# chaoyang223/UDA

Measured on AMD Instinct MI355X. Metric: TeraSort shuffle+merge GB/s whole-node, higher is better.
Workload: dtype bytes

## Files before the change

csrc/gpu/device_engine.cc:

```cpp
#include "device_engine.h"
#include "codec/colpack.h"
#include "device_ptr.h"
#include "hbm_ledger.h"
#include "merge_plan.h"
#include "sdma.h"
#include "uda/fault.h"
#include "uda/topology.h"
#include "uda/trace.h"

#include <rccl/rccl.h>
#include <unistd.h>

#include <algorithm>
#include <atomic>
#include <chrono>
#include <cstring>
#include <map>
#include <mutex>
#include <numeric>
#include <stdexcept>

#include "uda/log.h"
#include "uda/vint.h"
#include "uda/thread_name.h"
// ... 675 lines not shown
  HIP_CHECK(hipStreamWaitEvent(s, pb.planned, 0));
  KwayDesc kd = kp.kd;
  static const bool prof = std::getenv("UDA_KWAY_PROF") != nullptr;
  if (prof) {
    auto ensure = [](DeviceBuffer& b, size_t bytes) {
      if (b.size() < bytes) b.alloc_local(bytes + bytes / 8);
    };
    ensure(kw_prof_, (size_t)kp.ncells * 5 * 8);
    HIP_CHECK(hipMemsetAsync(kw_prof_.as(), 0, (size_t)kp.ncells * 5 * 8, s));
    kd.prof = kw_prof_.as<unsigned long long>();
  }
  HIP_CHECK(hipGetLastError());
  launch_kway_tiles(kd, kp.ncells, out, s);
  HIP_CHECK(hipGetLastError());
  HIP_CHECK(hipEventRecord(pb.used, s));
  pb.used_valid = true;
  if (prof) report_kway_phases(kd.prof, kp.ncells, s);
  last_passes_ = 1;
  return kp.total;
}

ShuffleJob::ShuffleJob(const ShuffleConfig& cfg) : cfg_(cfg) {
  if (cfg_.world < 1 || cfg_.rank < 0 || cfg_.rank >= cfg_.world)
    throw std::runtime_error("ShuffleJob: bad rank/world");
  if (cfg_.maps_per_rank < 1) throw std::runtime_error("ShuffleJob: maps_per_rank < 1");
  if (cfg_.rounds < 1) cfg_.rounds = 1;
  if (cfg_.reducers < 1) cfg_.reducers = 1;
  if (cfg_.pinned_slots < 2) cfg_.pinned_slots = 2;
  if (cfg_.d2h != "sdma" && cfg_.d2h != "hip") throw std::runtime_error("ShuffleJob: d2h must be sdma or hip");
  if (cfg_.store != "hbm" && cfg_.store != "host" && cfg_.store != "disk")
    throw std::runtime_error("unknown store tier " + cfg_.store);
  if (cfg_.delivery_pack != "auto" && cfg_.delivery_pack != "off")
    throw std::runtime_error("ShuffleJob: delivery_pack must be auto or off");
  pack_ = cfg_.deliver_host && cfg_.delivery_pack == "auto";
  if (const char* e = std::getenv("UDA_DELIVERY_PACK"))
    if (std::atoi(e) == 0) pack_ = false;
  R_ = cfg_.reducers;
  Q_ = cfg_.rounds;
  C_ = R_ * Q_;
  if ((int64_t)R_ * cfg_.world * cfg_.maps_per_rank > 65536)
    throw std::runtime_error("ShuffleJob: reducers * world * maps_per_rank must be <= 65536 (merge run index)");
  HIP_CHECK(hipSetDevice(cfg_.device));
  int lo_prio = 0, hi_prio = 0;
  HIP_CHECK(hipDeviceGetStreamPriorityRange(&lo_prio, &hi_prio));
  const bool spill = cfg_.store != "hbm";
  HIP_CHECK(hipStreamCreateWithPriority(&s_comm_, hipStreamNonBlocking, spill ? lo_prio : hi_prio));
  HIP_CHECK(hipStreamCreateWithPriority(&s_compute_, hipStreamNonBlocking, spill ? hi_prio : lo_prio));
  HIP_CHECK(hipStreamCreateWithFlags(&s_copy_, hipStreamNonBlocking));
  HIP_CHECK(hipStreamCreateWithFlags(&s_plan_, hipStreamNonBlocking));
  buf_records_ = std::max<int64_t>(1, cfg_.kv_buf_bytes / kTeraRecordBytes);
  const int64_t buf_bytes = buf_records_ * kTeraRecordBytes;
  piece_bytes_ = std::max<int64_t>(1, cfg_.d2h_piece_bytes / buf_bytes) * buf_bytes;
  ring_stride_ = pack_ ? std::max(piece_bytes_, colpack_bound(kTeraRecordBytes, piece_bytes_ / kTeraRecordBytes))
                       : piece_bytes_;
  merged_ev_.resize(kSlots);
  comm_ev_.resize(kSlots);
  sent_ev_.resize(2);
  for (auto& e : merged_ev_) HIP_CHECK(hipEventCreateWithFlags(&e, hipEventDisableTiming));
  for (auto& e : comm_ev_) HIP_CHECK(hipEventCreateWithFlags(&e, hipEventDisableTiming));
  for (auto& e : sent_ev_) HIP_CHECK(hipEventCreateWithFlags(&e, hipEventDisableTiming));
}

ShuffleJob::~ShuffleJob() {
  {
    std::lock_guard<std::mutex> g(mu_);
    stop_ = true;
// ... 15 lines not shown
    ring_ = nullptr;
    sdma_.reset();
  }
  exchange_.reset();
  if (s_copy_) (void)hipStreamDestroy(s_copy_);
  if (s_plan_) (void)hipStreamDestroy(s_plan_);
  if (s_comm_) (void)hipStreamDestroy(s_comm_);
  if (s_compute_) (void)hipStreamDestroy(s_compute_);
}

void ShuffleJob::init_comm(const std::string& uid) {
  if (cfg_.world == 1) return;
  HIP_CHECK(hipSetDevice(cfg_.device));
  exchange_ = make_rccl_exchange(cfg_.rank, cfg_.world, uid);
}

void ShuffleJob::init_local() {
  if (cfg_.world == 1) return;
  if (cfg_.local_group.empty()) throw std::runtime_error("init_local: config.local_group is empty");
  HIP_CHECK(hipSetDevice(cfg_.device));
  exchange_ = make_local_exchange(cfg_.local_group, cfg_.rank, cfg_.world);
}

void ShuffleJob::init_ipc(const std::string& name) {
  if (cfg_.world == 1) return;
  HIP_CHECK(hipSetDevice(cfg_.device));
  exchange_ = make_ipc_exchange(name, cfg_.rank, cfg_.world, cfg_.device);
}

std::string ShuffleJob::delivery_name() const {
  if (!cfg_.deliver_host) return "none";
  std::string name = sdma_ ? sdma_->describe() : "hip[numa=" + std::to_string(device_numa_node(cfg_.device)) + "]";
  name += " ring=" + ring_numa_;
  if (!pack_) return name + " pack=off";
  name += " pack=colbits";
  if (last_d2h_ratio_ >= 0) {
    char b[32];
    std::snprintf(b, sizeof(b), " d2h/in=%.3f", last_d2h_ratio_);
    name += b;
  }
  return name;
}

std::vector<ShuffleJob::PackPiece> ShuffleJob::round_pieces(const std::vector<int64_t>& group_recs) const {
  std::vector<PackPiece> v;
  int64_t goff = 0, doff = 0;
  for (int i = 0; i < R_; ++i) {
    const int64_t bytes = group_recs[i] * kTeraRecordBytes;
    for (int64_t off = 0; off < bytes;) {
      const int64_t len = std::min(piece_bytes_, bytes - off);
      const int64_t nrec = len / kTeraRecordBytes;
      v.push_back(PackPiece{goff + off, doff, nrec});
      doff += colpack_bound(kTeraRecordBytes, nrec);
      off += len;
    }
    goff += bytes;
  }
  return v;
}

void ShuffleJob::generate() {
  HIP_CHECK(hipSetDevice(cfg_.device));
  const int M = cfg_.maps_per_rank, W = cfg_.world;
  const int nruns = M * W;
  run_off_.assign(nruns, 0);
  run_nrec_.assign(nruns, 0);
// ... 576 lines not shown
      piece_sig_.resize(cfg_.pinned_slots);
      for (auto& sg : piece_sig_) sg = sdma_->make_signal();
    } else {
      ring_ = static_cast<uint8_t*>(hip_host_alloc_on_node(ring_bytes, device_numa_node(cfg_.device)));
      piece_ev_.resize(cfg_.pinned_slots);
      for (auto& e : piece_ev_) HIP_CHECK(hipEventCreateWithFlags(&e, hipEventDisableTiming));
    }
    for (size_t o = 0; o < ring_bytes; o += 4096) ring_[o] = 0;
    ring_numa_ = numa_residency(ring_);
    pinned_free_.assign(cfg_.pinned_slots, true);
    items_.assign(R_, {});
    eof_bufs_.clear();
    for (int i = 0; i < R_; ++i) eof_bufs_.emplace_back(new uint8_t[(size_t)cfg_.kv_buf_bytes + 16]);
    unpack_bufs_.clear();
    if (pack_) {
      const size_t one = (size_t)std::max(cfg_.kv_buf_bytes, buf_records_ * kTeraRecordBytes) + 16;
      for (int i = 0; i < R_; ++i) unpack_bufs_.emplace_back(new uint8_t[2 * one]);
    }
    copy_thr_ = std::thread([this] { name_thread("uda-copy"); copy_loop(); });
    for (int i = 0; i < R_; ++i) consumers_.emplace_back([this, i] { name_thread("uda-consume"); consume_loop(i); });
  }
  UDA_LOG(kInfo, "rank %d planned %d reducers x %d rounds, max round %ld records, delivery %s", cfg_.rank, R_, Q_,
          (long)max_round_records_, delivery_name().c_str());
}

void ShuffleJob::wait_exchange_ok() {
  if (exchange_) exchange_->check();
}

void ShuffleJob::copy_loop() {
  try {
    bind_thread_to_cpus(device_consumer_cpus(cfg_.device));
    HIP_CHECK(hipSetDevice(cfg_.device));
    for (;;) {
      RoundOut r;
      {
        std::unique_lock<std::mutex> lk(mu_);
        cv_.wait(lk, [&] { return stop_ || !round_q_.empty(); });
        if (stop_) return;
        r = std::move(round_q_.front());
        round_q_.pop_front();
      }
      HIP_CHECK(hipEventSynchronize(merged_ev_[r.slot]));
      const uint8_t* src = out_slots_[r.slot].as<uint8_t>();
      const bool last_round = (r.q == Q_ - 1);
      bool check;
      {
        std::lock_guard<std::mutex> g(mu_);
        check = step_check_delivery_;
      }
      if (check) {
        std::vector<RunDesc> gr(R_);
        int64_t o = 0, mx = 0;
        for (int i = 0; i < R_; ++i) {
          gr[i].base = src + o * kTeraRecordBytes;
          gr[i].nrec = r.group_recs[i];
          gr[i].nbytes = gr[i].nrec * kTeraRecordBytes;
          gr[i].offsets = nullptr;
          o += r.group_recs[i];
          mx = std::max(mx, r.group_recs[i]);
        }
        std::vector<uint64_t> ck(R_, 0);
        HIP_CHECK(hipMemcpyAsync(d_d2h_runs_.as(), gr.data(), (size_t)R_ * sizeof(RunDesc), hipMemcpyHostToDevice, s_copy_));
        launch_slice_checksums(d_d2h_runs_.as<RunDesc>(), R_, std::max<int64_t>(mx, 1),
                               d_d2h_ck_.as<unsigned long long>(), s_copy_);
        HIP_CHECK(hipGetLastError());
        HIP_CHECK(hipMemcpyAsync(ck.data(), d_d2h_ck_.as(), (size_t)R_ * 8, hipMemcpyDeviceToHost, s_copy_));
        HIP_CHECK(hipStreamSynchronize(s_copy_));
        std::lock_guard<std::mutex> g(mu_);
        for (int i = 0; i < R_; ++i) pre_d2h_ck_[(size_t)r.q * R_ + i] = ck[i];
      }
      std::vector<int> used;
      int64_t goff = 0;
      const std::vector<PackPiece> ppieces = pack_ ? round_pieces(r.group_recs) : std::vector<PackPiece>();
      const ColpackResult* pres = pack_ ? h_pack_results_[r.slot].as<ColpackResult>() : nullptr;
      size_t pi = 0;
      for (int i = 0; i < R_; ++i) {
        const int64_t bytes = r.group_recs[i] * kTeraRecordBytes;
        if (bytes == 0 && last_round) {
          {
            std::lock_guard<std::mutex> g(mu_);
            items_[i].push_back(Item{-1, 0, true, now_ms(), r.q});
          }
          cv_.notify_all();
        }
        for (int64_t off = 0; off < bytes;) {
          const int64_t len = std::min(piece_bytes_, bytes - off);
          int k = -1;
          {
            std::unique_lock<std::mutex> lk(mu_);
            cv_.wait(lk, [&] {
              if (stop_) return true;
              for (bool f : pinned_free_)
                if (f) return true;
              return false;
            });
            if (stop_) return;
            for (int x = 0; x < (int)pinned_free_.size(); ++x)
              if (pinned_free_[x]) {
                k = x;
                break;
              }
            pinned_free_[k] = false;
          }
          uint8_t* dst = ring_ + (int64_t)k * ring_stride_;
          const uint8_t* from = src + goff + off;
          int64_t copy_len = len;
          bool packed = false;
          if (pack_) {
            if (pi >= ppieces.size() || ppieces[pi].src_off != goff + off || ppieces[pi].nrec * kTeraRecordBytes != len)
              throw std::runtime_error("delivery_pack: piece list out of step with the copy loop");
            const ColpackResult pr = pres[pi];
            if (pr.packed) {
              if (pr.bytes < (int64_t)kColpackHeaderBytes || pr.bytes > colpack_bound(kTeraRecordBytes, ppieces[pi].nrec))
                throw std::runtime_error("delivery_pack: packed length outside the piece's region");
              packed = true;
              copy_len = pr.bytes;
              from = packed_slots_[r.slot].as<uint8_t>() + ppieces[pi].dst_off;
            }
            ++pi;
          }
          if (sdma_) {
            SdmaEngine::arm(piece_sig_[k], sdma_->parts((size_t)copy_len, cfg_.d2h_engines));
            sdma_->copy_d2h(dst, from, (size_t)copy_len, piece_sig_[k], cfg_.d2h_engines);
          } else {
            HIP_CHECK(hipMemcpyAsync(dst, from, (size_t)copy_len, hipMemcpyDeviceToHost, s_copy_));
            HIP_CHECK(hipEventRecord(piece_ev_[k], s_copy_));
          }
          off += len;
          used.push_back(k);
          {
            std::lock_guard<std::mutex> g(mu_);
            items_[i].push_back(Item{k, len, last_round && off >= bytes, now_ms(), r.q, packed, copy_len});
            step_d2h_bytes_ += copy_len;
            ++(packed ? step_packed_ : step_raw_);
          }
          cv_.notify_all();
        }
        goff += bytes;
      }
      for (int k : used) {
        if (sdma_)
          SdmaEngine::wait(piece_sig_[k]);
        else
          HIP_CHECK(hipEventSynchronize(piece_ev_[k]));
      }
      {
        std::lock_guard<std::mutex> g(mu_);
        out_free_[r.q] = 1;
      }
      cv_.notify_all();
    }
  } catch (const std::exception& e) {
    std::lock_guard<std::mutex> g(mu_);
    if (step_error_msg_.empty()) step_error_msg_ = std::string("delivery copy thread: ") + e.what();
    stop_ = true;
    cv_.notify_all();
  }
}

void ShuffleJob::consume_loop(int i) {
  try {
    bind_thread_to_cpus(device_consumer_cpus(cfg_.device));
    HIP_CHECK(hipSetDevice(cfg_.device));
    const int64_t buf_bytes = buf_records_ * kTeraRecordBytes;
    uint8_t* eb = eof_bufs_[i].get();
    const size_t unpack_one = (size_t)std::max(cfg_.kv_buf_bytes, buf_bytes) + 16;
    int64_t unpack_turn = 0;
    for (;;) {
      Item it;
      bool check;
      {
        std::unique_lock<std::mutex> lk(mu_);
        cv_.wait(lk, [&] { return stop_ || !items_[i].empty(); });
        if (stop_) return;
        it = items_[i].front();
        items_[i].pop_front();
        check = step_check_delivery_;
      }
      uint64_t got_ck = 0;
      int err = 0;
      int64_t nb = 0;
      double waited = 0;
      bool eof_sent = false;
      double unpack_ms = 0;
      if (it.pslot >= 0) {
        if (sdma_)
          SdmaEngine::wait(piece_sig_[it.pslot]);
        else
          HIP_CHECK(hipEventSynchronize(piece_ev_[it.pslot]));
        waited = now_ms() - it.issued_ms;
        const uint8_t* base = ring_ + (int64_t)it.pslot * ring_stride_;
        ColpackPiece pp;
        if (it.packed) {
          const char* why = "";
          if (!colpack_open(base, it.copied, kTeraRecordBytes, it.bytes / kTeraRecordBytes, &pp, &why) || !pp.packed)
            throw std::runtime_error(std::string("packed piece rejected: ") + (pp.hdr ? "not marked packed" : why));
        }
        if (check && !it.packed)
          for (int64_t off = 0; off + kTeraRecordBytes <= it.bytes; off += kTeraRecordBytes)
            got_ck += record_hash(base + off, kTeraRecordBytes);
        for (int64_t off = 0; off < it.bytes; off += buf_bytes) {
          const int64_t len = std::min(buf_bytes, it.bytes - off);
          const bool final_chunk = it.last && off + len >= it.bytes;
          if (it.packed) {
            uint8_t* stg = unpack_bufs_[i].get() + (size_t)(unpack_turn++ & 1) * unpack_one;
            if (check || (sink_ && !err)) {
              const double tu = now_ms();
              colpack_unpack(pp, off / kTeraRecordBytes, len / kTeraRecordBytes, stg);
              unpack_ms += now_ms() - tu;
            }
            if (check)
              for (int64_t o = 0; o + kTeraRecordBytes <= len; o += kTeraRecordBytes)
                got_ck += record_hash(stg + o, kTeraRecordBytes);
            if (final_chunk && len + kEofBytes <= cfg_.kv_buf_bytes) {
              stg[len] = 0xFF;
              stg[len + 1] = 0xFF;
              if (sink_ && !err) err = sink_(i, stg, len + kEofBytes);
              eof_sent = true;
            } else if (sink_ && !err) {
              err = sink_(i, stg, len);
            }
            ++nb;
            continue;
          }
          if (final_chunk && len + kEofBytes <= cfg_.kv_buf_bytes) {
            std::memcpy(eb, base + off, (size_t)len);
            eb[len] = 0xFF;
            eb[len + 1] = 0xFF;
            if (sink_ && !err) err = sink_(i, eb, len + kEofBytes);
            eof_sent = true;
          } else if (sink_ && !err) {
            err = sink_(i, base + off, len);
          }
          ++nb;
        }
      }
      if (it.last && !eof_sent) {
        eb[0] = 0xFF;
        eb[1] = 0xFF;
        if (sink_ && !err) err = sink_(i, eb, kEofBytes);
        ++nb;
      }
      {
        std::lock_guard<std::mutex> g(mu_);
        if (it.pslot >= 0) pinned_free_[it.pslot] = true;
        if (check && it.q >= 0 && it.q < Q_) delivered_ck_[(size_t)it.q * R_ + i] += got_ck;
        step_buffers_ += nb;
        step_d2h_ms_ += waited;
        step_unpack_ms_ += unpack_ms;
        if (err && !step_error_) step_error_ = err;
        if (it.last) ++eof_count_;
      }
      cv_.notify_all();
    }
  } catch (const std::exception& e) {
    std::lock_guard<std::mutex> g(mu_);
    if (step_error_msg_.empty()) step_error_msg_ = std::string("delivery consumer thread: ") + e.what();
    stop_ = true;
    cv_.notify_all();
  }
}

void ShuffleJob::refresh_plan() {
  const int M = cfg_.maps_per_rank, W = cfg_.world;
  const int nruns = M * W;
  const int64_t per = C_ + 1;
  for_run_batches([&](int r0, int nr, uint8_t* const* bases, const int64_t* nrec, const int* bset) {
    launch_split_fixed(bases, nrec, C_ > 1 ? d_bounds_.as<Elem>() : nullptr, bset, nr, C_ - 1,
                       d_split_out_.as<int64_t>() + (size_t)r0 * per, s_compute_);
  });
  std::vector<int64_t> pos((size_t)nruns * per);
  HIP_CHECK(hipMemcpyAsync(pos.data(), d_split_out_.as(), pos.size() * 8, hipMemcpyDeviceToHost, s_compute_));
  HIP_CHECK(hipStreamSynchronize(s_compute_));
  if (pos != split_pos_) throw std::runtime_error("replan: the map outputs changed since plan()");
  if (W == 1) return;
  const size_t n_per_peer = (size_t)Q_ * R_ * M;
  std::vector<int64_t> send((size_t)W * n_per_peer), recv((size_t)W * n_per_peer);
  for (int p = 0; p < W; ++p)
    for (int q = 0; q < Q_; ++q)
      for (int i = 0; i < R_; ++i)
        for (int m = 0; m < M; ++m) {
          const int r = m * W + p, c = i * Q_ + q;
          send[(size_t)p * n_per_peer + ((size_t)q * R_ + i) * M + m] = pos[(size_t)r * per + c + 1] - pos[(size_t)r * per + c];
        }
// ... 46 lines not shown
        ++st.pre_d2h_errors;
        note(first[3], "output slot changed between the merge and its D2H", q, i, pre_d2h[(size_t)q * R_ + i], merged);
      }
      if (deliv[(size_t)q * R_ + i] != merged) {
        ++st.delivery_errors;
        note(first[4], "consumer received other bytes than the merge wrote", q, i, deliv[(size_t)q * R_ + i], merged);
      }
    }
  }
  st.diag.clear();
  for (const auto& f : first)
    if (!f.empty()) st.diag += (st.diag.empty() ? "" : "; ") + f;
}

StepStats ShuffleJob::run_step(bool validate) {
  trace::Range tr_step("uda.step");
  HIP_CHECK(hipSetDevice(cfg_.device));
  if (!merger_) throw std::runtime_error("run_step before plan()");
  StepStats st;
  st.validated = validate;
  const double t0 = now_ms();
  const int M = cfg_.maps_per_rank, W = cfg_.world, me = cfg_.rank;
  const bool deliver = cfg_.deliver_host;
  {
    std::lock_guard<std::mutex> g(mu_);
    if (stop_) throw std::runtime_error("delivery pipeline stopped: " + step_error_msg_);
    out_free_.assign(Q_, 0);
    eof_count_ = 0;
    step_buffers_ = 0;
    step_error_ = 0;
    step_d2h_ms_ = 0;
    step_d2h_bytes_ = step_packed_ = step_raw_ = 0;
    step_unpack_ms_ = 0;
    step_check_delivery_ = validate && cfg_.check_delivery && deliver;
    pre_d2h_ck_.assign((size_t)Q_ * R_, 0);
    delivered_ck_.assign((size_t)Q_ * R_, 0);
  }
  std::vector<hipEvent_t> ev(4 * (size_t)Q_);
  for (auto& e : ev) HIP_CHECK(hipEventCreate(&e));
  unsigned long long* vstats = d_validate_.as<unsigned long long>();
  Elem* vprev = reinterpret_cast<Elem*>(d_validate_.as<uint8_t>() + 64);
  Elem* vlast = vprev + R_;
  std::vector<bool> has_prev(R_, false);
  if (validate) {
    HIP_CHECK(hipMemsetAsync(d_validate_.as(), 0, 64, s_compute_));
    HIP_CHECK(hipMemsetAsync(d_diag_.as(), 0, (size_t)Q_ * diag_stride() * 8, s_compute_));
  }
  if (cfg_.replan) {
    const double tp = now_ms();
    refresh_plan();
    st.plan_ms = now_ms() - tp;
  }

  auto wait_until = [&](const std::function<bool()>& ready) {
    std::unique_lock<std::mutex> lk(mu_);
    while (!cv_.wait_for(lk, std::chrono::milliseconds(100), [&] { return ready() || stop_; })) {
      if (exchange_) {
        lk.unlock();
        wait_exchange_ok();
        lk.lock();
      }
    }
    if (stop_) throw std::runtime_error("delivery pipeline failed: " + step_error_msg_);
  };

  const bool staged_send = W > 1 && spilled();
// ... 230 lines not shown
        if (g > 0) {
          launch_validate_fixed(out + goff * kTeraRecordBytes, g, vprev + i, has_prev[i] ? 1 : 0, vlast + i, vstats,
                                s_compute_, dg + 4 + i);
          HIP_CHECK(hipMemcpyAsync(vprev + i, vlast + i, sizeof(Elem), hipMemcpyDeviceToDevice, s_compute_));
          has_prev[i] = true;
        }
        goff += g;
      }
      check_inputs(1);
    }
    HIP_CHECK(hipEventRecord(ev[4 * q + 3], s_compute_));
    if (pack_ && deliver && pack_n_[q] > 0) {
      launch_colpack(d_pack_pieces_[q].as<ColpackPieceDesc>(), pack_n_[q], pack_max_nrec_[q], kTeraRecordBytes,
                     buf_records_, d_pack_table_.as<uint32_t>(), d_pack_results_[slot].as<ColpackResult>(), s_compute_);
      HIP_CHECK(hipGetLastError());
      HIP_CHECK(hipMemcpyAsync(h_pack_results_[slot].as(), d_pack_results_[slot].as(),
                               (size_t)pack_n_[q] * sizeof(ColpackResult), hipMemcpyDeviceToHost, s_compute_));
    }
    HIP_CHECK(hipEventRecord(merged_ev_[slot], s_compute_));
    if (sdma_stage) {
      std::lock_guard<std::mutex> g(mu_);
      merge_recorded[q] = 1;
      cv_.notify_all();
    }
    st.records += n;
    if (deliver) {
      {
        std::lock_guard<std::mutex> g(mu_);
        round_q_.push_back(RoundOut{q, slot, rp.group_recs});
      }
      cv_.notify_all();
    }
  }
  if (deliver) wait_until([&] { return eof_count_ == R_; });
  if (exchange_) exchange_->wait(s_comm_);
  HIP_CHECK(hipStreamSynchronize(s_compute_));
  HIP_CHECK(hipStreamSynchronize(s_comm_));
  HIP_CHECK(hipStreamSynchronize(s_copy_));
  if (stage_thr.joinable()) stage_thr.join();
  if (exchange_) exchange_->quiesce();
  st.wall_ms = now_ms() - t0;
  st.stage_ms = stage_ms;
  for (int q = 0; q < Q_; ++q) {
    float a = 0, b = 0;
    if (staged() && hipEventElapsedTime(&a, ev[4 * q + 0], ev[4 * q + 1]) == hipSuccess) st.comm_ms += a;
    if (hipEventElapsedTime(&b, ev[4 * q + 2], ev[4 * q + 3]) == hipSuccess) st.merge_ms += b;
    st.round_comm_ms.push_back(a);
    st.round_merge_ms.push_back(b);
  }
  static const bool round_trace = std::getenv("UDA_ROUND_TRACE") != nullptr;
  if (round_trace && staged()) {
    std::string line = "[round trace ms: comm start-end | merge start-end]";
    for (int q = 0; q < Q_; ++q) {
      float t[4] = {0, 0, 0, 0};
      for (int k = 0; k < 4; ++k) (void)hipEventElapsedTime(&t[k], ev[0], ev[4 * q + k]);
      char b[96];
      snprintf(b, sizeof(b), " q%d %.0f-%.0f|%.0f-%.0f", q, t[0], t[1], t[2], t[3]);
      line += b;
    }
    fprintf(stderr, "%s\n", line.c_str());
  }
  for (auto e : ev) (void)hipEventDestroy(e);
  st.d2h_ms = step_d2h_ms_;
  st.bytes_in = st.records * kTeraRecordBytes;
  st.buffers = step_buffers_;
  {
    std::lock_guard<std::mutex> g(mu_);
    st.d2h_bytes = step_d2h_bytes_;
    st.packed_pieces = step_packed_;
    st.raw_pieces = step_raw_;
    st.unpack_ms = step_unpack_ms_;
  }
  if (deliver && st.bytes_in > 0) last_d2h_ratio_ = (double)st.d2h_bytes / (double)st.bytes_in;
  if (validate) {
    unsigned long long v[3];
    HIP_CHECK(hipMemcpy(v, vstats, sizeof(v), hipMemcpyDeviceToHost));
    st.order_errors = (int64_t)v[0];
    st.checksum = v[1];
    st.exchange_errors = W > 1 ? (int64_t)v[2] : 0;
    localize_mismatch(st);
  }
  st.bad_layout = merger_->bad_layout();
  if (step_error_) throw std::runtime_error("delivery sink reported error " + std::to_string(step_error_));
  return st;
}

}
}
```

csrc/gpu/device_engine.h:

```cpp
#pragma once
#include <hip/hip_runtime.h>

#include <atomic>
#include <condition_variable>
#include <cstdint>
#include <deque>
#include <functional>
#include <map>
#include <memory>
#include <mutex>
#include <string>
#include <thread>
#include <vector>

#include "exchange.h"
#include "kernels.h"
#include "disk_store.h"
#include "sdma.h"

namespace uda {
namespace gpu {

void hip_check(hipError_t e, const char* what, const char* file, int line);
#define HIP_CHECK(x) ::uda::gpu::hip_check((x), #x, __FILE__, __LINE__)
#define HIP_PENDING(where) ::uda::gpu::hip_check(hipGetLastError(), "a call before " where, __FILE__, __LINE__)

class DeviceBuffer {
 public:
  DeviceBuffer() = default;
  explicit DeviceBuffer(size_t bytes, bool resident = false) { alloc(bytes, resident); }
  ~DeviceBuffer();
  DeviceBuffer(const DeviceBuffer&) = delete;
  DeviceBuffer& operator=(const DeviceBuffer&) = delete;
  DeviceBuffer(DeviceBuffer&& o) noexcept { take(o); }
  DeviceBuffer& operator=(DeviceBuffer&& o) noexcept {
    if (this != &o) {
      reset();
      take(o);
    }
    return *this;
  }
  void alloc(size_t bytes, bool resident = false) { alloc_impl(bytes, resident, true); }
  void alloc_local(size_t bytes) { alloc_impl(bytes, false, false); }
  void reset();
  template <typename T = uint8_t>
  T* as() const {
    return reinterpret_cast<T*>(ptr_);
// ... 138 lines not shown
  PlanBufs pbufs_[2];
  int next_pslot_ = 0;
  std::vector<Slot> slots_;
  int next_slot_ = 0;
  int last_passes_ = 0;
  size_t slot_bytes_ = 0;
};

using SinkFn = std::function<int(int reducer, const uint8_t* buf, int64_t len)>;

struct ShuffleConfig {
  int device = 0;
  int rank = 0;
  int world = 1;
  int maps_per_rank = 32;
  int64_t records_per_map = 1 << 20;
  int rounds = 8;
  int reducers = 1;
  uint64_t seed = 0x5eed;
  int64_t kv_buf_bytes = 1 << 20;
  int64_t d2h_piece_bytes = 128ll << 20;
  int pinned_slots = 16;
  int d2h_engines = 1;
  std::string d2h = "sdma";
  bool deliver_host = true;
  bool validate = false;
  std::string local_group;
  std::string store = "hbm";
  std::string local_dirs;
  bool replan = false;
  bool map_sort = false;
  bool check_delivery = false;
  std::string delivery_pack = "auto";
};

struct StepStats {
  double wall_ms = 0;
  double comm_ms = 0;
  double merge_ms = 0;
  double d2h_ms = 0;
  double wait_out_ms = 0;
  double plan_ms = 0;
  double stage_ms = 0;
  int64_t bytes_in = 0;
  int64_t records = 0;
  int64_t bytes_sent = 0;
  int64_t bytes_h2d = 0;
  int64_t buffers = 0;
  int64_t d2h_bytes = 0;
  int64_t packed_pieces = 0;
  int64_t raw_pieces = 0;
  double unpack_ms = 0;
  int merge_passes = 0;
  bool validated = false;
  int64_t order_errors = -1;
  uint64_t checksum = 0;
  int64_t exchange_errors = -1;
  bool bad_layout = false;
  int64_t pre_merge_errors = -1;
  int64_t own_errors = -1;
  int64_t merge_errors = -1;
  int64_t pre_d2h_errors = -1;
  int64_t delivery_errors = -1;
  std::string diag;
  std::vector<double> round_comm_ms, round_merge_ms;
};

class ShuffleJob {
 public:
  explicit ShuffleJob(const ShuffleConfig& cfg);
  ~ShuffleJob();

  const ShuffleConfig& config() const { return cfg_; }
  void init_comm(const std::string& uid);
  void init_local();
  void init_ipc(const std::string& name);
  void generate();
  std::vector<std::vector<uint64_t>> sample_keys(int64_t every);
  void set_bounds(const std::vector<uint64_t>& bounds);
  void plan();
  void set_sink(SinkFn sink) { sink_ = std::move(sink); }
  StepStats run_step(bool validate);
  void refresh_plan();

  std::vector<uint64_t> local_dest_checksums() const { return dest_checksum_; }
// ... 116 lines not shown
  std::string ring_numa_;
  std::vector<hsa_signal_t> piece_sig_;
  std::vector<hipEvent_t> piece_ev_;
  struct RoundOut {
    int q;
    int slot;
    std::vector<int64_t> group_recs;
  };
  struct Item {
    int pslot;
    int64_t bytes;
    bool last;
    double issued_ms;
    int q;
    bool packed = false;
    int64_t copied = 0;
  };
  std::mutex mu_;
  std::condition_variable cv_;
  std::deque<RoundOut> round_q_;
  std::vector<std::deque<Item>> items_;
  std::vector<bool> pinned_free_;
  std::vector<int> out_free_;
  std::thread copy_thr_;
  std::vector<std::thread> consumers_;
  bool stop_ = false;
  int eof_count_ = 0;
  int64_t step_buffers_ = 0;
  int step_error_ = 0;
  std::string step_error_msg_;
  double step_d2h_ms_ = 0;
  int64_t step_d2h_bytes_ = 0, step_packed_ = 0, step_raw_ = 0;
  double step_unpack_ms_ = 0;
  SinkFn sink_;
  std::vector<std::unique_ptr<uint8_t[]>> eof_bufs_;
  std::vector<std::unique_ptr<uint8_t[]>> unpack_bufs_;
};

std::string nccl_unique_id();
int device_count();

hipStream_t pooled_stream(int priority = 0);
int64_t device_guard_violations();
void return_stream(hipStream_t s);
void prewarm_streams(int device, int n);

}
}
```

csrc/gpu/sdma.cc:

```cpp
#include "sdma.h"
#include "uda/topology.h"

#include <hip/hip_runtime.h>
#include <sched.h>
#include <sys/mman.h>
#include <sys/syscall.h>
#include <unistd.h>

#include <algorithm>
#include <cstdio>
#include <cstdlib>
#include <cstring>
#include <fstream>
#include <sstream>
#include <stdexcept>
#include <mutex>
#include <thread>
#include <atomic>
#include <map>
#include <unordered_map>
#include <vector>

#include "uda/log.h"

// ... 455 lines not shown
    hsa_check(s, "agents_allow_access");
  }
  return p;
}

void SdmaEngine::free_host(void* p) {
  if (!p) return;
  PinnedShare ps;
  if (pinned_share_of(p, 1, &ps))
    pinned_host_free(p);
  else
    (void)hsa_amd_memory_pool_free(p);
}

hsa_signal_t SdmaEngine::make_signal() {
  hsa_signal_t s;
  hsa_check(hsa_signal_create(0, 0, nullptr, &s), "signal_create");
  return s;
}

void SdmaEngine::destroy_signal(hsa_signal_t s) {
  if (s.handle) (void)hsa_signal_destroy(s);
}

void SdmaEngine::arm(hsa_signal_t s, int64_t parts) { hsa_signal_store_screlease(s, parts); }
void SdmaEngine::add(hsa_signal_t s, int64_t parts) { hsa_signal_add_screlease(s, parts); }

void SdmaEngine::wait(hsa_signal_t s) {
  const hsa_signal_value_t v =
      hsa_signal_wait_scacquire(s, HSA_SIGNAL_CONDITION_LT, 1, UINT64_MAX, HSA_WAIT_STATE_BLOCKED);
  if (v < 0) throw std::runtime_error("SDMA copy reported an error (completion signal < 0)");
}

int SdmaEngine::parts(size_t bytes, int ways) const {
  if (bytes == 0) return 0;
  if (ways < 1) ways = 1;
  const size_t min_part = (size_t)8 << 20;
  int n = (int)std::min<size_t>((size_t)ways, (bytes + min_part - 1) / min_part);
  return n < 1 ? 1 : n;
}

int SdmaEngine::copy_d2h(void* dst_host, const void* src_dev, size_t bytes, hsa_signal_t sig, int ways) {
  const int n = parts(bytes, ways);
  if (n == 0) return 0;
  size_t per = (bytes + n - 1) / n;
  per = (per + 4095) & ~(size_t)4095;
  size_t off = 0;
  int issued = 0;
  for (int k = 0; k < n && off < bytes; ++k) {
    const size_t len = std::min(per, bytes - off);
    void* d = static_cast<uint8_t*>(dst_host) + off;
    const void* s = static_cast<const uint8_t*>(src_dev) + off;
    hsa_status_t st = HSA_STATUS_ERROR;
    if (!engine_ids_.empty()) {
      const uint32_t eng = engine_ids_[(size_t)(next_engine_.fetch_add(1) & 0x7fffffff) % engine_ids_.size()];
      st = hsa_amd_memory_async_copy_on_engine(d, cpu_, s, gpu_, len, 0, nullptr, sig,
                                               (hsa_amd_sdma_engine_id_t)eng, false);
    }
    if (st != HSA_STATUS_SUCCESS) st = hsa_amd_memory_async_copy(d, cpu_, s, gpu_, len, 0, nullptr, sig);
    hsa_check(st, "memory_async_copy (D2H)");
    off += len;
    ++issued;
  }
  for (int k = issued; k < n; ++k) hsa_signal_subtract_screlease(sig, 1);
  return n;
}
// ... 27 lines not shown
```

csrc/gpu/sdma.h:

```cpp
#pragma once
#include <hsa/hsa.h>
#include <hsa/hsa_ext_amd.h>

#include <atomic>
#include <cstdint>
#include <map>
#include <mutex>
#include <string>
#include <vector>

namespace uda {
namespace gpu {

class SdmaEngine {
 public:
  static SdmaEngine& for_device(int device);
  explicit SdmaEngine(int device);
  ~SdmaEngine();
  SdmaEngine(const SdmaEngine&) = delete;
  SdmaEngine& operator=(const SdmaEngine&) = delete;

  void* alloc_host(size_t bytes);
  void free_host(void* p);
  void* acquire_ring(size_t bytes);
  void release_ring(void* p, size_t bytes);

  hsa_signal_t make_signal();
  void destroy_signal(hsa_signal_t s);
  int copy_d2h(void* dst_host, const void* src_dev, size_t bytes, hsa_signal_t sig, int ways);
  int parts(size_t bytes, int ways) const;
  void copy_h2d(void* dst_dev, const void* src_host, size_t bytes, hsa_signal_t sig);
  static void arm(hsa_signal_t s, int64_t parts);
  static void add(hsa_signal_t s, int64_t parts);
  static void wait(hsa_signal_t s);

  void warm(void* dev_scratch);
  int numa_node() const { return numa_node_; }
  int engines() const { return (int)engine_ids_.size(); }
  std::string describe() const;

 private:
  hsa_agent_t gpu_{}, cpu_{};
  hsa_amd_memory_pool_t host_pool_{};
  std::vector<uint32_t> engine_ids_;
  uint32_t h2d_engine_ = 0;
  int numa_node_ = -1;
  std::atomic<int> next_engine_{0};
  bool hsa_inited_ = false;
  std::mutex ring_mu_;
  std::multimap<size_t, void*> ring_cache_;
};

int device_numa_node(int device);
void bind_thread_to_numa(int node);
std::vector<int> device_consumer_cpus(int device);
void* pinned_host_alloc(size_t bytes, int node = -1);
void pinned_host_free(void* p);
void* hip_host_alloc_on_node(size_t bytes, int node);
struct PinnedShare {
  int fd = -1;
  uint64_t id = 0;
  size_t offset = 0, region_bytes = 0;
  int numa_node = -1;
};
void set_pinned_shareable(bool on);
bool pinned_share_of(const void* p, size_t len, PinnedShare* out);
std::string numa_residency(const void* p);
// ... 4 lines not shown
```

csrc/python/bindings.cc:

```cpp
#include <map>
#include <memory>
#include <condition_variable>
#include <mutex>
#include <pybind11/functional.h>
#include <pybind11/numpy.h>
#include <pybind11/pybind11.h>
#include <pybind11/stl.h>

#include <fcntl.h>
#include <unistd.h>

#include <atomic>
#include <chrono>
#include <cstring>

#include "block_decoder.h"
#include "device_engine.h"
#include "device_ptr.h"
#include "mof_cache.h"
#include "consumer/reduce_task.h"
#include "service/merge_service.h"
#include "exchange.h"
#include "api_bench.h"
#include "generic_merger.h"
// ... 20 lines not shown
#include <atomic>
#include <thread>

namespace py = pybind11;
using namespace uda;

namespace {

struct GpuNoise {
  std::atomic<bool> stop{false};
  std::thread thr;
  std::atomic<int64_t> ops{0};
};
GpuNoise* g_noise = nullptr;

py::dict stats_to_dict(const gpu::StepStats& s) {
  py::dict d;
  d["wall_ms"] = s.wall_ms;
  d["comm_ms"] = s.comm_ms;
  d["plan_ms"] = s.plan_ms;
  d["merge_ms"] = s.merge_ms;
  d["d2h_ms"] = s.d2h_ms;
  d["wait_out_ms"] = s.wait_out_ms;
  d["stage_ms"] = s.stage_ms;
  d["bytes_in"] = s.bytes_in;
  d["records"] = s.records;
  d["bytes_sent"] = s.bytes_sent;
  d["bytes_h2d"] = s.bytes_h2d;
  d["buffers"] = s.buffers;
  d["d2h_bytes"] = s.d2h_bytes;
  d["packed_pieces"] = s.packed_pieces;
  d["raw_pieces"] = s.raw_pieces;
  d["unpack_ms"] = s.unpack_ms;
  d["merge_passes"] = s.merge_passes;
  d["order_errors"] = s.order_errors;
  d["checksum"] = s.checksum;
  d["exchange_errors"] = s.exchange_errors;
  d["validated"] = s.validated;
  d["bad_layout"] = s.bad_layout;
  d["pre_merge_errors"] = s.pre_merge_errors;
  d["own_errors"] = s.own_errors;
  d["merge_errors"] = s.merge_errors;
  d["pre_d2h_errors"] = s.pre_d2h_errors;
  d["delivery_errors"] = s.delivery_errors;
  d["diag"] = s.diag;
  d["round_comm_ms"] = s.round_comm_ms;
  d["round_merge_ms"] = s.round_merge_ms;
  return d;
}

gpu::ShuffleConfig config_from_dict(const py::dict& d) {
  gpu::ShuffleConfig c;
  auto get = [&](const char* k, auto& field) {
    if (d.contains(k)) field = d[k].cast<std::decay_t<decltype(field)>>();
  };
  get("device", c.device);
  get("rank", c.rank);
  get("world", c.world);
  get("maps_per_rank", c.maps_per_rank);
  get("records_per_map", c.records_per_map);
  get("rounds", c.rounds);
  get("reducers", c.reducers);
  get("seed", c.seed);
  get("kv_buf_bytes", c.kv_buf_bytes);
  get("d2h_piece_bytes", c.d2h_piece_bytes);
  get("pinned_slots", c.pinned_slots);
  get("d2h_engines", c.d2h_engines);
  get("d2h", c.d2h);
  get("deliver_host", c.deliver_host);
  get("validate", c.validate);
  get("local_group", c.local_group);
  get("store", c.store);
  get("local_dirs", c.local_dirs);
  get("replan", c.replan);
  get("map_sort", c.map_sort);
  get("check_delivery", c.check_delivery);
  get("delivery_pack", c.delivery_pack);
  return c;
}

struct PyBridge {
  py::object fetch_over, data_from_uda, get_path, get_conf, log, failure;
  uda_handle* h = nullptr;
  std::vector<std::shared_ptr<std::string>> keep;

  static PyBridge* self(void* ctx) { return static_cast<PyBridge*>(ctx); }
  static void t_fetch_over(void* ctx) {
    py::gil_scoped_acquire g;
    try {
      if (!self(ctx)->fetch_over.is_none()) self(ctx)->fetch_over();
    } catch (py::error_already_set& e) {
      e.discard_as_unraisable("fetch_over");
    }
  }
  static int t_data(void* ctx, const void* buf, int32_t len) {
    py::gil_scoped_acquire g;
    try {
      if (self(ctx)->data_from_uda.is_none()) return 0;
      py::memoryview mv = py::memoryview::from_memory(const_cast<void*>(buf), (py::ssize_t)len, true);
      py::object r = self(ctx)->data_from_uda(mv);
      mv.attr("release")();
      return r.is_none() ? 0 : r.cast<int>();
    } catch (py::error_already_set& e) {
      e.discard_as_unraisable("data_from_uda");
      return -1;
    }
  }
  static int t_get_path(void* ctx, const char* job, const char* map, int32_t reduce, uda_index_record* out) {
    py::gil_scoped_acquire g;
    try {
// ... 1450 lines not shown
```

uda_amd/models/terasort.py:

```python
from __future__ import annotations

import dataclasses
import os
import sys
import secrets
import time

import numpy as np

from .._native import native
from ..parallel.dist import DistContext
from ..parallel.plan import round_bounds

RECORD_BYTES = 104
TERAGEN_ROW_BYTES = 100


@dataclasses.dataclass
class TeraSortConfig:
    rows_per_gpu: int = 1_250_000_000
    maps_per_rank: int = 32
    rounds: int = 16
    seed: int = 0x5EED
    kv_buf_bytes: int = 1 << 20
    reducers: int = 1
    d2h_piece_bytes: int = 128 << 20
    pinned_slots: int = 16
    d2h_engines: int = 1
    d2h: str = "sdma"
    deliver_host: bool = True
    validate: bool = False
    sample_every: int = 4096
    store: str = "hbm"
    local_dirs: str = "/tmp"
    replan: bool = False
    map_sort: bool = False
    check_delivery: bool = False
    delivery_pack: str = "auto"
    exchange: str = "ipc"


class TeraSortShuffle:
    def __init__(self, ctx: DistContext, cfg: TeraSortConfig, device: int | None = None):
        self.ctx = ctx
        self.cfg = cfg
        self.device = ctx.local_rank if device is None else device
        n = native()
        records_per_map = max(1, cfg.rows_per_gpu // cfg.maps_per_rank)
        self.records_per_map = records_per_map
        self.job = n.ShuffleJob(dict(
            device=self.device, rank=ctx.rank, world=ctx.world,
            maps_per_rank=cfg.maps_per_rank, records_per_map=records_per_map,
            rounds=cfg.rounds, reducers=cfg.reducers, seed=cfg.seed, kv_buf_bytes=cfg.kv_buf_bytes,
            d2h_piece_bytes=cfg.d2h_piece_bytes, pinned_slots=cfg.pinned_slots,
            d2h_engines=cfg.d2h_engines, d2h=cfg.d2h, deliver_host=cfg.deliver_host,
            validate=cfg.validate, store=cfg.store, local_dirs=cfg.local_dirs, replan=cfg.replan,
            map_sort=cfg.map_sort, check_delivery=cfg.check_delivery,
        delivery_pack=cfg.delivery_pack))
        self.sink = n.J2CSink(cfg.reducers, cfg.kv_buf_bytes)
        self.sampler = None
        self.sample_index = []
        self.expected_checksum = None
        self.expected_records = None
        self.setup_s = {}

    def setup(self) -> None:
        n = native()
        t0 = time.perf_counter()
        if self.ctx.world > 1:
            if self.cfg.exchange == "ipc" and not self._ipc_preflight():
                if os.environ.get("UDA_IPC_FALLBACK", "1") == "0":
                    raise RuntimeError(f"IPC exchange preflight failed ({self.ipc_fallback}); the job stops here "
                                       "(UDA_IPC_FALLBACK=0)")
                if self.ctx.rank == 0:
                    print(f"uda: IPC exchange preflight failed, shuffling over RCCL ({self.ipc_fallback})",
                          file=sys.stderr, flush=True)
                self.cfg.exchange = "rccl"
            if self.cfg.exchange == "ipc":
                name = f"uda.{os.getpid()}.{secrets.token_hex(6)}".encode() if self.ctx.rank == 0 else None
                self.job.init_ipc(self.ctx.broadcast_bytes(name).decode())
            elif self.cfg.exchange == "rccl":
                uid = n.nccl_unique_id() if self.ctx.rank == 0 else None
                uid = self.ctx.broadcast_bytes(uid)
                self.job.init_comm(uid)
            else:
                raise ValueError(f"unknown exchange {self.cfg.exchange!r}")
        t1 = time.perf_counter()
        self.job.generate()
        t2 = time.perf_counter()
        local = self.job.sample_keys(self.cfg.sample_every)
        gathered = self.ctx.all_gather_object([np.asarray(a) for a in local])
# ... 86 lines not shown
        raise AssertionError(f"records {stats['records']} != expected {expected_records}")
    if stats["bad_layout"]:
        raise AssertionError("non-TeraSort record layout seen by the merge")
    if "consumer_records" in stats:
        if list(stats["consumer_records"]) != list(reducer_records):
            raise AssertionError(f"consumers parsed {stats['consumer_records']} records, expected {reducer_records}")
        if any(stats["consumer_errors"]):
            raise AssertionError(f"consumer framing errors {stats['consumer_errors']}")
        if not all(stats["consumer_eof"]):
            raise AssertionError("a reducer did not receive its EOF marker")
    if stats["validated"]:
        if stats["order_errors"] != 0:
            raise AssertionError(f"{stats['order_errors']} out-of-order records")
        if stats["exchange_errors"] != 0:
            raise AssertionError(f"{stats['exchange_errors']} received slices differ from what their sender sent")
        for k in ("pre_merge_errors", "own_errors", "merge_errors", "pre_d2h_errors", "delivery_errors"):
            if stats.get(k, 0) > 0:
                raise AssertionError(f"{k} {stats[k]}: {stats.get('diag', '')}")
        if stats["checksum"] != expected_checksum:
            raise AssertionError("checksum mismatch " + stats.get("diag", ""))


def make_local_group(world: int, cfg: TeraSortConfig, device: int = 0, group: str = "local"):

    n = native()
    records_per_map = max(1, cfg.rows_per_gpu // cfg.maps_per_rank)
    jobs = [n.ShuffleJob(dict(
        device=device, rank=r, world=world, maps_per_rank=cfg.maps_per_rank,
        records_per_map=records_per_map, rounds=cfg.rounds, reducers=cfg.reducers, seed=cfg.seed,
        kv_buf_bytes=cfg.kv_buf_bytes, d2h_piece_bytes=cfg.d2h_piece_bytes, pinned_slots=cfg.pinned_slots,
        d2h_engines=cfg.d2h_engines, d2h=cfg.d2h, deliver_host=cfg.deliver_host, validate=cfg.validate,
        local_group=group, store=cfg.store, local_dirs=cfg.local_dirs, replan=cfg.replan,
        map_sort=cfg.map_sort, check_delivery=cfg.check_delivery,
        delivery_pack=cfg.delivery_pack))
        for r in range(world)]
    for j in jobs:
        j.init_local()
        j.generate()
    local = [j.sample_keys(cfg.sample_every) for j in jobs]
    per_dest = []
    for d in range(world):
        parts = [np.asarray(s[d]) for s in local if np.asarray(s[d]).size]
        per_dest.append(np.concatenate(parts) if parts else np.zeros((0, 2), np.uint64))
    bounds = np.ascontiguousarray(round_bounds(per_dest, cfg.rounds * cfg.reducers).reshape(-1))
    for j in jobs:
        j.set_bounds(bounds)
    run_collective(jobs, lambda j: j.plan())
    ck = [sum(j.local_dest_checksums()[d] for j in jobs) % (1 << 64) for d in range(world)]
    rec = [sum(j.local_dest_records()[d] for j in jobs) for d in range(world)]
    return jobs, ck, rec


def run_collective(jobs, fn):
    import threading

    out = [None] * len(jobs)
    err = []

    def work(i):
        try:
            out[i] = fn(jobs[i])
        except BaseException as e:
            err.append(e)

    ts = [threading.Thread(target=work, args=(i,)) for i in range(len(jobs))]
    for t in ts:
        t.start()
# ... 6 lines not shown
```

Measured before the change: 82.98.

## Interleave D2H delivery pieces round-robin across reducers and add link-idle instrumentation

The copy loop now issues device-to-host pieces round-robin across reducers by default, instead of draining one reducer fully before moving to the next. The goal is to keep every consumer thread fed at once so unpacking runs in parallel with the copies and less time is spent waiting on one reducer's ring slots. It also adds timing counters (link idle, ring wait, consume time, tail), a polling wait that detects when the link goes idle, and a stricter end-of-step wait on the last round's slot. These add some locking and bookkeeping overhead, and the final wait may lengthen the step slightly.

```diff
diff --git a/csrc/gpu/delivery_order.h b/csrc/gpu/delivery_order.h
--- /dev/null
+++ b/csrc/gpu/delivery_order.h
@@ -0,0 +1,61 @@
+#pragma once
+#include <algorithm>
+#include <string>
+#include <vector>
+
+namespace uda {
+namespace gpu {
+
+enum class DeliveryOrder { kInterleave, kReducer };
+
+struct DeliveryStep {
+  int reducer;
+  int piece;
+};
+
+inline bool parse_delivery_order(const std::string& s, DeliveryOrder* out) {
+  if (s == "interleave") {
+    *out = DeliveryOrder::kInterleave;
+    return true;
+  }
+  if (s == "reducer") {
+    *out = DeliveryOrder::kReducer;
+    return true;
+  }
+  return false;
+}
+
+inline const char* delivery_order_token(DeliveryOrder o) { return o == DeliveryOrder::kInterleave ? "rr" : "reducer"; }
+
+inline std::vector<DeliveryStep> delivery_order(const std::vector<int>& pieces_per_reducer, DeliveryOrder order) {
+  std::vector<DeliveryStep> v;
+  const int R = (int)pieces_per_reducer.size();
+  size_t total = 0;
+  int most = 0;
+  for (int n : pieces_per_reducer) {
+    total += (size_t)std::max(n, 0);
+    most = std::max(most, n);
+  }
+  v.reserve(total);
+  if (order == DeliveryOrder::kReducer) {
+    for (int i = 0; i < R; ++i)
+      for (int p = 0; p < pieces_per_reducer[i]; ++p) v.push_back(DeliveryStep{i, p});
+  } else {
+    for (int p = 0; p < most; ++p)
+      for (int i = 0; i < R; ++i)
+        if (p < pieces_per_reducer[i]) v.push_back(DeliveryStep{i, p});
+  }
+  return v;
+}
+
+inline int same_reducer_run_max(const std::vector<DeliveryStep>& steps) {
+  int best = 0, run = 0;
+  for (size_t k = 0; k < steps.size(); ++k) {
+    run = (k > 0 && steps[k].reducer == steps[k - 1].reducer) ? run + 1 : 1;
+    best = std::max(best, run);
+  }
+  return best;
+}
+
+}
+}
diff --git a/csrc/gpu/device_engine.cc b/csrc/gpu/device_engine.cc
--- a/csrc/gpu/device_engine.cc
+++ b/csrc/gpu/device_engine.cc
@@ -731,6 +731,8 @@
     throw std::runtime_error("unknown store tier " + cfg_.store);
   if (cfg_.delivery_pack != "auto" && cfg_.delivery_pack != "off")
     throw std::runtime_error("ShuffleJob: delivery_pack must be auto or off");
+  if (!parse_delivery_order(cfg_.delivery_order, &order_))
+    throw std::runtime_error("ShuffleJob: delivery_order must be interleave or reducer");
   pack_ = cfg_.deliver_host && cfg_.delivery_pack == "auto";
   if (const char* e = std::getenv("UDA_DELIVERY_PACK"))
     if (std::atoi(e) == 0) pack_ = false;
@@ -812,6 +814,7 @@
   if (!cfg_.deliver_host) return "none";
   std::string name = sdma_ ? sdma_->describe() : "hip[numa=" + std::to_string(device_numa_node(cfg_.device)) + "]";
   name += " ring=" + ring_numa_;
+  name += std::string(" order=") + delivery_order_token(order_);
   if (!pack_) return name + " pack=off";
   name += " pack=colbits";
   if (last_d2h_ratio_ >= 0) {
@@ -1454,6 +1457,8 @@
   try {
     bind_thread_to_cpus(device_consumer_cpus(cfg_.device));
     HIP_CHECK(hipSetDevice(cfg_.device));
+    int newest = -1;
+    double idle_since = -1;
     for (;;) {
       RoundOut r;
       {
@@ -1463,6 +1468,7 @@
         r = std::move(round_q_.front());
         round_q_.pop_front();
       }
+      if (r.q == 0) idle_since = -1;
       HIP_CHECK(hipEventSynchronize(merged_ev_[r.slot]));
       const uint8_t* src = out_slots_[r.slot].as<uint8_t>();
       const bool last_round = (r.q == Q_ - 1);
@@ -1493,73 +1499,106 @@
         for (int i = 0; i < R_; ++i) pre_d2h_ck_[(size_t)r.q * R_ + i] = ck[i];
       }
       std::vector<int> used;
-      int64_t goff = 0;
       const std::vector<PackPiece> ppieces = pack_ ? round_pieces(r.group_recs) : std::vector<PackPiece>();
       const ColpackResult* pres = pack_ ? h_pack_results_[r.slot].as<ColpackResult>() : nullptr;
-      size_t pi = 0;
-      for (int i = 0; i < R_; ++i) {
+      std::vector<int64_t> goff(R_, 0);
+      std::vector<int> npieces(R_, 0), first_piece(R_, 0);
+      {
+        int64_t o = 0;
+        int n = 0;
+        for (int i = 0; i < R_; ++i) {
+          const int64_t bytes = r.group_recs[i] * kTeraRecordBytes;
+          goff[i] = o;
+          first_piece[i] = n;
+          npieces[i] = (int)((bytes + piece_bytes_ - 1) / piece_bytes_);
+          o += bytes;
+          n += npieces[i];
+        }
+      }
+      if (last_round) {
+        bool any = false;
+        {
+          std::lock_guard<std::mutex> g(mu_);
+          for (int i = 0; i < R_; ++i)
+            if (npieces[i] == 0) {
+              items_[i].push_back(Item{-1, 0, true, now_ms(), r.q});
+              any = true;
+            }
+        }
+        if (any) cv_.notify_all();
+      }
+      const std::vector<DeliveryStep> order = delivery_order(npieces, order_);
+      const int run_max = same_reducer_run_max(order);
+      for (const DeliveryStep& ds : order) {
+        const int i = ds.reducer;
         const int64_t bytes = r.group_recs[i] * kTeraRecordBytes;
-        if (bytes == 0 && last_round) {
-          {
-            std::lock_guard<std::mutex> g(mu_);
-            items_[i].push_back(Item{-1, 0, true, now_ms(), r.q});
+        const int64_t off = (int64_t)ds.piece * piece_bytes_;
+        const int64_t len = std::min(piece_bytes_, bytes - off);
+        const bool final_piece = ds.piece == npieces[i] - 1;
+        int k = -1;
+        double ring_wait = 0;
+        {
+          std::unique_lock<std::mutex> lk(mu_);
+          const double tw = now_ms();
+          bool waited = false;
+          for (;;) {
+            if (stop_) return;
+            for (int x = 0; x < (int)pinned_free_.size() && k < 0; ++x)
+              if (pinned_free_[x]) k = x;
+            if (k >= 0) break;
+            waited = true;
+            if (idle_since >= 0 || newest < 0) {
+              cv_.wait(lk);
+              continue;
+            }
+            cv_.wait_for(lk, std::chrono::microseconds(200));
+            lk.unlock();
+            const bool landed = sdma_ ? SdmaEngine::done(piece_sig_[newest]) : hipEventQuery(piece_ev_[newest]) == hipSuccess;
+            if (landed) idle_since = now_ms();
+            lk.lock();
           }
-          cv_.notify_all();
+          pinned_free_[k] = false;
+          if (waited) ring_wait = now_ms() - tw;
         }
-        for (int64_t off = 0; off < bytes;) {
-          const int64_t len = std::min(piece_bytes_, bytes - off);
-          int k = -1;
-          {
-            std::unique_lock<std::mutex> lk(mu_);
-            cv_.wait(lk, [&] {
-              if (stop_) return true;
-              for (bool f : pinned_free_)
-                if (f) return true;
-              return false;
-            });
-            if (stop_) return;
-            for (int x = 0; x < (int)pinned_free_.size(); ++x)
-              if (pinned_free_[x]) {
-                k = x;
-                break;
-              }
-            pinned_free_[k] = false;
+        uint8_t* dst = ring_ + (int64_t)k * ring_stride_;
+        const uint8_t* from = src + goff[i] + off;
+        int64_t copy_len = len;
+        bool packed = false;
+        if (pack_) {
+          const size_t pi = (size_t)first_piece[i] + (size_t)ds.piece;
+          if (pi >= ppieces.size() || ppieces[pi].src_off != goff[i] + off || ppieces[pi].nrec * kTeraRecordBytes != len)
+            throw std::runtime_error("delivery_pack: piece list out of step with the copy loop");
+          const ColpackResult pr = pres[pi];
+          if (pr.packed) {
+            if (pr.bytes < (int64_t)kColpackHeaderBytes || pr.bytes > colpack_bound(kTeraRecordBytes, ppieces[pi].nrec))
+              throw std::runtime_error("delivery_pack: packed length outside the piece's region");
+            packed = true;
+            copy_len = pr.bytes;
+            from = packed_slots_[r.slot].as<uint8_t>() + ppieces[pi].dst_off;
           }
-          uint8_t* dst = ring_ + (int64_t)k * ring_stride_;
-          const uint8_t* from = src + goff + off;
-          int64_t copy_len = len;
-          bool packed = false;
-          if (pack_) {
-            if (pi >= ppieces.size() || ppieces[pi].src_off != goff + off || ppieces[pi].nrec * kTeraRecordBytes != len)
-              throw std::runtime_error("delivery_pack: piece list out of step with the copy loop");
-            const ColpackResult pr = pres[pi];
-            if (pr.packed) {
-              if (pr.bytes < (int64_t)kColpackHeaderBytes || pr.bytes > colpack_bound(kTeraRecordBytes, ppieces[pi].nrec))
-                throw std::runtime_error("delivery_pack: packed length outside the piece's region");
-              packed = true;
-              copy_len = pr.bytes;
-              from = packed_slots_[r.slot].as<uint8_t>() + ppieces[pi].dst_off;
-            }
-            ++pi;
-          }
-          if (sdma_) {
-            SdmaEngine::arm(piece_sig_[k], sdma_->parts((size_t)copy_len, cfg_.d2h_engines));
-            sdma_->copy_d2h(dst, from, (size_t)copy_len, piece_sig_[k], cfg_.d2h_engines);
-          } else {
-            HIP_CHECK(hipMemcpyAsync(dst, from, (size_t)copy_len, hipMemcpyDeviceToHost, s_copy_));
-            HIP_CHECK(hipEventRecord(piece_ev_[k], s_copy_));
-          }
-          off += len;
-          used.push_back(k);
-          {
-            std::lock_guard<std::mutex> g(mu_);
-            items_[i].push_back(Item{k, len, last_round && off >= bytes, now_ms(), r.q, packed, copy_len});
-            step_d2h_bytes_ += copy_len;
-            ++(packed ? step_packed_ : step_raw_);
-          }
-          cv_.notify_all();
         }
-        goff += bytes;
+        const double t_issue = now_ms();
+        if (sdma_) {
+          SdmaEngine::arm(piece_sig_[k], sdma_->parts((size_t)copy_len, cfg_.d2h_engines));
+          sdma_->copy_d2h(dst, from, (size_t)copy_len, piece_sig_[k], cfg_.d2h_engines);
+        } else {
+          HIP_CHECK(hipMemcpyAsync(dst, from, (size_t)copy_len, hipMemcpyDeviceToHost, s_copy_));
+          HIP_CHECK(hipEventRecord(piece_ev_[k], s_copy_));
+        }
+        used.push_back(k);
+        newest = k;
+        {
+          std::lock_guard<std::mutex> g(mu_);
+          items_[i].push_back(Item{k, len, last_round && final_piece, now_ms(), r.q, packed, copy_len});
+          step_d2h_bytes_ += copy_len;
+          ++(packed ? step_packed_ : step_raw_);
+          if (step_first_issue_ms_ < 0) step_first_issue_ms_ = t_issue;
+          else if (idle_since >= 0) step_link_idle_ms_ += t_issue - idle_since;
+          step_ring_wait_ms_ += ring_wait;
+          step_run_max_ = std::max(step_run_max_, run_max);
+        }
+        idle_since = -1;
+        cv_.notify_all();
       }
       for (int k : used) {
         if (sdma_)
@@ -1567,9 +1606,11 @@
         else
           HIP_CHECK(hipEventSynchronize(piece_ev_[k]));
       }
+      if (!used.empty() && idle_since < 0) idle_since = now_ms();
       {
         std::lock_guard<std::mutex> g(mu_);
         out_free_[r.q] = 1;
+        if (!used.empty()) step_last_land_ms_ = idle_since;
       }
       cv_.notify_all();
     }
@@ -1606,12 +1647,14 @@
       double waited = 0;
       bool eof_sent = false;
       double unpack_ms = 0;
+      double t_hand = -1;
       if (it.pslot >= 0) {
         if (sdma_)
           SdmaEngine::wait(piece_sig_[it.pslot]);
         else
           HIP_CHECK(hipEventSynchronize(piece_ev_[it.pslot]));
-        waited = now_ms() - it.issued_ms;
+        t_hand = now_ms();
+        waited = t_hand - it.issued_ms;
         const uint8_t* base = ring_ + (int64_t)it.pslot * ring_stride_;
         ColpackPiece pp;
         if (it.packed) {
@@ -1671,8 +1714,13 @@
         step_buffers_ += nb;
         step_d2h_ms_ += waited;
         step_unpack_ms_ += unpack_ms;
+        const double t_done = now_ms();
+        if (t_hand >= 0) step_consume_ms_[i] += t_done - t_hand;
         if (err && !step_error_) step_error_ = err;
-        if (it.last) ++eof_count_;
+        if (it.last) {
+          ++eof_count_;
+          step_last_eof_ms_ = std::max(step_last_eof_ms_, t_done);
+        }
       }
       cv_.notify_all();
     }
@@ -1785,6 +1833,11 @@
     step_d2h_ms_ = 0;
     step_d2h_bytes_ = step_packed_ = step_raw_ = 0;
     step_unpack_ms_ = 0;
+    step_t0_ms_ = t0;
+    step_first_issue_ms_ = step_last_land_ms_ = step_last_eof_ms_ = -1;
+    step_link_idle_ms_ = step_ring_wait_ms_ = 0;
+    step_run_max_ = 0;
+    step_consume_ms_.assign(R_, 0.0);
     step_check_delivery_ = validate && cfg_.check_delivery && deliver;
     pre_d2h_ck_.assign((size_t)Q_ * R_, 0);
     delivered_ck_.assign((size_t)Q_ * R_, 0);
@@ -2081,7 +2134,7 @@
       cv_.notify_all();
     }
   }
-  if (deliver) wait_until([&] { return eof_count_ == R_; });
+  if (deliver) wait_until([&] { return eof_count_ == R_ && out_free_[Q_ - 1]; });
   if (exchange_) exchange_->wait(s_comm_);
   HIP_CHECK(hipStreamSynchronize(s_compute_));
   HIP_CHECK(hipStreamSynchronize(s_comm_));
@@ -2119,6 +2172,15 @@
     st.packed_pieces = step_packed_;
     st.raw_pieces = step_raw_;
     st.unpack_ms = step_unpack_ms_;
+    st.link_idle_ms = step_link_idle_ms_;
+    st.ring_wait_ms = step_ring_wait_ms_;
+    st.first_issue_ms = step_first_issue_ms_ >= 0 ? step_first_issue_ms_ - step_t0_ms_ : 0;
+    st.tail_ms = step_last_land_ms_ >= 0 && step_last_eof_ms_ >= 0 ? std::max(0.0, step_last_eof_ms_ - step_last_land_ms_) : 0;
+    for (double c : step_consume_ms_) {
+      st.consume_ms += c;
+      st.consume_max_ms = std::max(st.consume_max_ms, c);
+    }
+    st.same_reducer_run_max = step_run_max_;
   }
   if (deliver && st.bytes_in > 0) last_d2h_ratio_ = (double)st.d2h_bytes / (double)st.bytes_in;
   if (validate) {
diff --git a/csrc/gpu/device_engine.h b/csrc/gpu/device_engine.h
--- a/csrc/gpu/device_engine.h
+++ b/csrc/gpu/device_engine.h
@@ -13,6 +13,7 @@
 #include <thread>
 #include <vector>
 
+#include "delivery_order.h"
 #include "exchange.h"
 #include "kernels.h"
 #include "disk_store.h"
@@ -217,6 +218,7 @@
   bool map_sort = false;
   bool check_delivery = false;
   std::string delivery_pack = "auto";
+  std::string delivery_order = "interleave";
 };
 
 struct StepStats {
@@ -236,6 +238,13 @@
   int64_t packed_pieces = 0;
   int64_t raw_pieces = 0;
   double unpack_ms = 0;
+  double link_idle_ms = 0;
+  double ring_wait_ms = 0;
+  double first_issue_ms = 0;
+  double tail_ms = 0;
+  double consume_ms = 0;
+  double consume_max_ms = 0;
+  int same_reducer_run_max = 0;
   int merge_passes = 0;
   bool validated = false;
   int64_t order_errors = -1;
@@ -418,6 +427,11 @@
   double step_d2h_ms_ = 0;
   int64_t step_d2h_bytes_ = 0, step_packed_ = 0, step_raw_ = 0;
   double step_unpack_ms_ = 0;
+  DeliveryOrder order_ = DeliveryOrder::kInterleave;
+  double step_t0_ms_ = 0, step_first_issue_ms_ = -1, step_last_land_ms_ = -1, step_last_eof_ms_ = -1;
+  double step_link_idle_ms_ = 0, step_ring_wait_ms_ = 0;
+  int step_run_max_ = 0;
+  std::vector<double> step_consume_ms_;
   SinkFn sink_;
   std::vector<std::unique_ptr<uint8_t[]>> eof_bufs_;
   std::vector<std::unique_ptr<uint8_t[]>> unpack_bufs_;
diff --git a/csrc/gpu/sdma.cc b/csrc/gpu/sdma.cc
--- a/csrc/gpu/sdma.cc
+++ b/csrc/gpu/sdma.cc
@@ -511,6 +511,8 @@
   if (v < 0) throw std::runtime_error("SDMA copy reported an error (completion signal < 0)");
 }
 
+bool SdmaEngine::done(hsa_signal_t s) { return hsa_signal_load_scacquire(s) < 1; }
+
 int SdmaEngine::parts(size_t bytes, int ways) const {
   if (bytes == 0) return 0;
   if (ways < 1) ways = 1;
diff --git a/csrc/gpu/sdma.h b/csrc/gpu/sdma.h
--- a/csrc/gpu/sdma.h
+++ b/csrc/gpu/sdma.h
@@ -33,6 +33,7 @@
   static void arm(hsa_signal_t s, int64_t parts);
   static void add(hsa_signal_t s, int64_t parts);
   static void wait(hsa_signal_t s);
+  static bool done(hsa_signal_t s);
 
   void warm(void* dev_scratch);
   int numa_node() const { return numa_node_; }
diff --git a/csrc/python/bindings.cc b/csrc/python/bindings.cc
--- a/csrc/python/bindings.cc
+++ b/csrc/python/bindings.cc
@@ -76,6 +76,13 @@
   d["packed_pieces"] = s.packed_pieces;
   d["raw_pieces"] = s.raw_pieces;
   d["unpack_ms"] = s.unpack_ms;
+  d["link_idle_ms"] = s.link_idle_ms;
+  d["ring_wait_ms"] = s.ring_wait_ms;
+  d["first_issue_ms"] = s.first_issue_ms;
+  d["tail_ms"] = s.tail_ms;
+  d["consume_ms"] = s.consume_ms;
+  d["consume_max_ms"] = s.consume_max_ms;
+  d["same_reducer_run_max"] = s.same_reducer_run_max;
   d["merge_passes"] = s.merge_passes;
   d["order_errors"] = s.order_errors;
   d["checksum"] = s.checksum;
@@ -120,6 +127,7 @@
   get("map_sort", c.map_sort);
   get("check_delivery", c.check_delivery);
   get("delivery_pack", c.delivery_pack);
+  get("delivery_order", c.delivery_order);
   return c;
 }
 
diff --git a/uda_amd/models/terasort.py b/uda_amd/models/terasort.py
--- a/uda_amd/models/terasort.py
+++ b/uda_amd/models/terasort.py
@@ -37,6 +37,7 @@
     map_sort: bool = False
     check_delivery: bool = False
     delivery_pack: str = "auto"
+    delivery_order: str = "interleave"
     exchange: str = "ipc"
 
 
@@ -56,7 +57,7 @@
             d2h_engines=cfg.d2h_engines, d2h=cfg.d2h, deliver_host=cfg.deliver_host,
             validate=cfg.validate, store=cfg.store, local_dirs=cfg.local_dirs, replan=cfg.replan,
             map_sort=cfg.map_sort, check_delivery=cfg.check_delivery,
-        delivery_pack=cfg.delivery_pack))
+            delivery_pack=cfg.delivery_pack, delivery_order=cfg.delivery_order))
         self.sink = n.J2CSink(cfg.reducers, cfg.kv_buf_bytes)
         self.sampler = None
         self.sample_index = []
@@ -209,7 +210,7 @@
         d2h_engines=cfg.d2h_engines, d2h=cfg.d2h, deliver_host=cfg.deliver_host, validate=cfg.validate,
         local_group=group, store=cfg.store, local_dirs=cfg.local_dirs, replan=cfg.replan,
         map_sort=cfg.map_sort, check_delivery=cfg.check_delivery,
-        delivery_pack=cfg.delivery_pack))
+        delivery_pack=cfg.delivery_pack, delivery_order=cfg.delivery_order))
         for r in range(world)]
     for j in jobs:
         j.init_local()
```

Result: slower. 77.89 (-6.1%).
